# batra-mlp-lab/visdial

Measured on AMD Instinct MI355X. Metric: QA-rounds/sec training mn-att-ques-im-hist+disc (batch 20x10x100), higher is better.
Workload: dtype f32 operands and results; the option recurrence multiplies the EXACT 3-way bf16 split of both operands (9 bf16 MFMA products per fp32 product, f32 accumulate: fp32-grade, errors at the f32 MFMA's own level) -- its two step kernels and its weight-gradient contraction; f32 MFMA (v_mfma_f32_32x32x2_f32

## Files before the change

visdial_amd/csrc/gemm_ops.hip:

```cpp
#include "gemm_core.h"
#include "split_core.h"

using CfgBigDB = GemmCfg<4, 1, 4, 32>;
using CfgBig = GemmCfg<4, 1, 4, 16, 0, 3>;
using CfgSmall = GemmCfg<1, 4, 1, 32, 0, 3>;

static inline bool use_small(int M, int N) {
  return (long)vd_cdiv(M, CfgBig::BM) * vd_cdiv(N, CfgBig::BN) < 48;
}

static int check_align(const void* p, long ld, const char* what) {
  if (((uintptr_t)p & 15) != 0 || (ld & 3) != 0) {
    vd_set_error("%s: pointer must be 16-byte aligned and leading dimension a multiple of 4 (ld=%ld)", what, ld);
    return VD_ERR_ARG;
  }
  return VD_OK;
}

__global__ void colsum_kernel(const float* __restrict__ X, long ld, int M, int N, int rows_per_block,
                              float* __restrict__ out) {
  const int col = blockIdx.x * blockDim.x + threadIdx.x;
  if (col >= N) return;
  const int r0 = blockIdx.y * rows_per_block;
  const int r1 = min(M, r0 + rows_per_block);
// ... 69 lines not shown
  constexpr int TILE = 8192;
  char* const lds = reinterpret_cast<char*>(smem);
  const int wg = xcd_remap(blockIdx.x, gridDim.x);
  const int tile_n = wg % tiles_n, tile_m = (wg / tiles_n) % tiles_m, split = wg / (tiles_n * tiles_m);
  const int ks = split * kchunk, ke = min(K, ks + kchunk);
  const int nk = ke > ks ? (ke - ks) / 32 : 0;
  const int lane = threadIdx.x & 63;
  const int wm = __builtin_amdgcn_readfirstlane((int)threadIdx.x >> 6);
  const int m0 = tile_m * 128, n0 = tile_n * 128;

  f32x16 acc[4];
#pragma unroll
  for (int j = 0; j < 4; ++j)
#pragma unroll
    for (int r = 0; r < 16; ++r) acc[j][r] = 0.f;

  const int key = (lane & 7) >> 1, col = (lane >> 3) * 16 + (lane & 1) * 8;
  unsigned voffa[2], voffb[2];
#pragma unroll
  for (int i = 0; i < 2; ++i) {
    const int krow = (i * 4 + wm) * 4 + key;
    voffa[i] = (unsigned)(((long)krow * M + m0 + col) * 2);
    voffb[i] = (unsigned)(((long)krow * N + n0 + col) * 2);
  }
  const unsigned lds0 = (unsigned)(uintptr_t)lds;
  auto issue = [&](int kt, int buf) {
    const float* ak = reinterpret_cast<const float*>(A + (long)(ks + kt * 32) * M);
    const float* bk = reinterpret_cast<const float*>(B + (long)(ks + kt * 32) * N);
#pragma unroll
    for (int i = 0; i < 2; ++i) glds16(voffb[i], bk, lds0 + buf * 2 * TILE + TILE + (i * 4 + wm) * 1024);
#pragma unroll
    for (int i = 0; i < 2; ++i) glds16(voffa[i], ak, lds0 + buf * 2 * TILE + (i * 4 + wm) * 1024);
  };
  const int g = lane >> 4, li = lane & 15;
  const int frag = ((g >> 1) * 2) * 1024 + (g & 1) * 128 + li * 8;

  if (nk > 0) {
    issue(0, 0);
    if (nk > 1) issue(1, 1);
    int buf = 0;
    for (int kt = 0; kt < nk; ++kt) {
      if (kt + 1 < nk) asm volatile("s_waitcnt vmcnt(4)" ::: "memory");
      else asm volatile("s_waitcnt vmcnt(0)" ::: "memory");
      asm volatile("s_barrier" ::: "memory");
      if (kt + 2 < nk) issue(kt + 2, buf == 0 ? 2 : buf - 1);
      const char* ta = lds + buf * 2 * TILE;
      const char* tb = ta + TILE;
#pragma unroll
      for (int st = 0; st < 2; ++st) {
        const vd_bf16x8 a8 = tr_read8(ta, frag + st * 4096 + wm * 256);
        vd_bf16x8 b8[4];
#pragma unroll
        for (int j = 0; j < 4; ++j) b8[j] = tr_read8(tb, frag + st * 4096 + j * 256);
#pragma unroll
        for (int j = 0; j < 4; ++j) acc[j] = __builtin_amdgcn_mfma_f32_32x32x16_bf16(a8, b8[j], acc[j], 0, 0, 0);
      }
      buf = buf == 2 ? 0 : buf + 1;
    }
  }
#pragma unroll
  for (int j = 0; j < 4; ++j) {
    const int c = n0 + j * 32 + (lane & 31);
#pragma unroll
    for (int r = 0; r < 16; ++r) {
      const int row = m0 + wm * 32 + mfma_row(r, lane);
      unsafeAtomicAdd(C + (long)row * ldc + c, acc[j][r]);
    }
  }
}

template <int NBUF>
__global__ void __launch_bounds__(512)
gemm_bf16_tn_tr256_kernel(const vd_bf16_bits* __restrict__ A, const vd_bf16_bits* __restrict__ B, float* __restrict__ C, long ldc,
                          int M, int N, int K, int kchunk, int tiles_m, int tiles_n) {
  extern __shared__ __attribute__((aligned(16))) float smem[];
  constexpr int TILE = 16384;
  char* const lds = reinterpret_cast<char*>(smem);
  const int wg = xcd_remap(blockIdx.x, gridDim.x);
  const int tile_n = wg % tiles_n, tile_m = (wg / tiles_n) % tiles_m, split = wg / (tiles_n * tiles_m);
  const int ks = split * kchunk, ke = min(K, ks + kchunk);
  const int nk = ke > ks ? (ke - ks) / 32 : 0;
  const int lane = threadIdx.x & 63;
  const int w = __builtin_amdgcn_readfirstlane((int)threadIdx.x >> 6);
  const int wm = w & 3, wn = w >> 2;
  const int m0 = tile_m * 256, n0 = tile_n * 256;

  f32x16 acc[2][4];
#pragma unroll
  for (int i = 0; i < 2; ++i)
#pragma unroll
    for (int j = 0; j < 4; ++j)
#pragma unroll
      for (int r = 0; r < 16; ++r) acc[i][j][r] = 0.f;

  unsigned voffa[2], voffb[2];
#pragma unroll
  for (int i = 0; i < 2; ++i) {
    const int krow = (i * 8 + w) * 2 + (lane >> 5);
    const int cb = ((lane & 31) * 16) ^ ((krow & 3) << 6);
    voffa[i] = (unsigned)(((long)krow * M + m0) * 2 + cb);
    voffb[i] = (unsigned)(((long)krow * N + n0) * 2 + cb);
  }
  const unsigned lds0 = (unsigned)(uintptr_t)lds;
  auto issue = [&](int kt, int buf) {
    const float* ak = reinterpret_cast<const float*>(A + (long)(ks + kt * 32) * M);
    const float* bk = reinterpret_cast<const float*>(B + (long)(ks + kt * 32) * N);
#pragma unroll
    for (int i = 0; i < 2; ++i) glds16(voffb[i], bk, lds0 + buf * 2 * TILE + TILE + (i * 8 + w) * 1024);
#pragma unroll
    for (int i = 0; i < 2; ++i) glds16(voffa[i], ak, lds0 + buf * 2 * TILE + (i * 8 + w) * 1024);
  };
  const int g = lane >> 4, li = lane & 15;
  const int frag = (g >> 1) * 4096 + (li >> 2) * 512 + (g & 1) * 32 + (li & 3) * 8;
  int xa[2], xb[4];
#pragma unroll
  for (int i = 0; i < 2; ++i) xa[i] = frag + (((wm * 2 + i) ^ (li >> 2)) << 6);
#pragma unroll
  for (int j = 0; j < 4; ++j) xb[j] = frag + (((wn * 4 + j) ^ (li >> 2)) << 6);
  auto rd8 = [&](const char* base, int off) {
    typedef __attribute__((address_space(3))) vd_s16x4* lds_p;
    union {
      vd_s16x4 h[2];
      vd_bf16x8 v;
    } u;
    u.h[0] = __builtin_amdgcn_ds_read_tr16_b64_v4i16((lds_p)(base + off));
    u.h[1] = __builtin_amdgcn_ds_read_tr16_b64_v4i16((lds_p)(base + off + 2048));
    return u.v;
  };

  struct Frags {
    vd_bf16x8 a[2], b[4];
  };
  auto read_step = [&](Frags& f, int buf, int st) {
    const char* ta = lds + buf * 2 * TILE;
    const char* tb = ta + TILE;
#pragma unroll
    for (int i = 0; i < 2; ++i) f.a[i] = rd8(ta, xa[i] + st * 8192);
#pragma unroll
    for (int j = 0; j < 4; ++j) f.b[j] = rd8(tb, xb[j] + st * 8192);
  };
  auto mfma_step = [&](const Frags& f) {
#pragma unroll
    for (int i = 0; i < 2; ++i)
#pragma unroll
      for (int j = 0; j < 4; ++j) acc[i][j] = __builtin_amdgcn_mfma_f32_32x32x16_bf16(f.a[i], f.b[j], acc[i][j], 0, 0, 0);
  };
  auto wait_tiles_in_flight = [&](int later) {
    if (later >= 3) asm volatile("s_waitcnt vmcnt(12)" ::: "memory");
    else if (later == 2) asm volatile("s_waitcnt vmcnt(8)" ::: "memory");
    else if (later == 1) asm volatile("s_waitcnt vmcnt(4)" ::: "memory");
    else asm volatile("s_waitcnt vmcnt(0)" ::: "memory");
  };
  if (nk > 0) {
#pragma unroll
    for (int i = 0; i < NBUF - 1; ++i)
      if (i < nk) issue(i, i);
    wait_tiles_in_flight(min(NBUF - 2, nk - 1));
    asm volatile("s_barrier" ::: "memory");
    Frags f0, f1;
    read_step(f0, 0, 0);
    int buf = 0;
    for (int kt = 0; kt < nk; ++kt) {
      const int nbuf = buf == NBUF - 1 ? 0 : buf + 1;
      read_step(f1, buf, 1);
      mfma_step(f0);
      if (kt + 1 < nk) {
        wait_tiles_in_flight(min(NBUF - 3, nk - 2 - kt));
        asm volatile("s_barrier" ::: "memory");
        if (kt + NBUF - 1 < nk) issue(kt + NBUF - 1, buf == 0 ? NBUF - 1 : buf - 1);
        read_step(f0, nbuf, 0);
      }
      mfma_step(f1);
      buf = nbuf;
    }
  }
#pragma unroll
  for (int i = 0; i < 2; ++i)
#pragma unroll
    for (int j = 0; j < 4; ++j) {
      const int c = n0 + wn * 128 + j * 32 + (lane & 31);
#pragma unroll
      for (int r = 0; r < 16; ++r) {
        const int row = m0 + wm * 64 + i * 32 + mfma_row(r, lane);
        unsafeAtomicAdd(C + (long)row * ldc + c, acc[i][j][r]);
      }
    }
}

static int launch_gemm_bf16_tn_tr256(const vd_bf16_bits* A, const vd_bf16_bits* B, float* C, long ldc, int M, int N, int K,
                                     hipStream_t stream) {
  const int tiles_m = M / 256, tiles_n = N / 256;
  long splits = vd_cdiv(256, (long)tiles_m * tiles_n);
  int kchunk = vd_cdiv(vd_cdiv(K, splits), 32) * 32;
  if (kchunk < 32) kchunk = 32;
  splits = vd_cdiv(K, kchunk);
  static bool attr_set = false;
#ifndef VD_TR256_NBUF
#define VD_TR256_NBUF 3
#endif
  constexpr int NBUF = VD_TR256_NBUF;
  const int lds = NBUF * 2 * 16384;
  if (!attr_set) {
    VD_HIP(hipFuncSetAttribute(reinterpret_cast<const void*>(gemm_bf16_tn_tr256_kernel<NBUF>),
                               hipFuncAttributeMaxDynamicSharedMemorySize, lds));
    attr_set = true;
  }
  hipLaunchKernelGGL(gemm_bf16_tn_tr256_kernel<NBUF>, dim3((unsigned)(tiles_m * tiles_n * splits)), dim3(512), lds, stream, A, B, C,
                     ldc, M, N, K, kchunk, tiles_m, tiles_n);
  VD_LAUNCH_CHECK();
  return VD_OK;
}

static int launch_gemm_bf16_tn_tr(const vd_bf16_bits* A, const vd_bf16_bits* B, float* C, long ldc, int M, int N, int K,
                                  hipStream_t stream) {
  const int tiles_m = M / 128, tiles_n = N / 128;
  long splits = vd_cdiv(768, (long)tiles_m * tiles_n);
  int kchunk = vd_cdiv(vd_cdiv(K, splits), 32) * 32;
  if (kchunk < 32) kchunk = 32;
  splits = vd_cdiv(K, kchunk);
  static bool attr_set = false;
  const int lds = 3 * 2 * 8192;
  if (!attr_set) {
    VD_HIP(hipFuncSetAttribute(reinterpret_cast<const void*>(gemm_bf16_tn_tr_kernel),
                               hipFuncAttributeMaxDynamicSharedMemorySize, lds));
    attr_set = true;
  }
  hipLaunchKernelGGL(gemm_bf16_tn_tr_kernel, dim3((unsigned)(tiles_m * tiles_n * splits)), dim3(256), lds, stream, A, B, C,
                     ldc, M, N, K, kchunk, tiles_m, tiles_n);
  VD_LAUNCH_CHECK();
  return VD_OK;
}

extern "C" {

int vd_gemm_nt(const float* A, int64_t lda, const float* W, int64_t ldw, const float* bias, float* C,
               int64_t ldc, int M, int N, int K, int act, int accumulate, void* stream) {
  VD_CHECK_ARG(A && W && C && M >= 0 && N >= 0 && K >= 0 && K % 4 == 0, "vd_gemm_nt: bad args M=%d N=%d K=%d", M,
               N, K);
  if (int rc = check_align(A, lda, "vd_gemm_nt A")) return rc;
  if (int rc = check_align(W, ldw, "vd_gemm_nt W")) return rc;
  SrcRow a{A, lda}, b{W, ldw};
  hipStream_t s = (hipStream_t)stream;
  if (use_small(M, N)) {
    EpiStore<1> e{C, ldc, bias, act, accumulate};
    return launch_gemm<CfgSmall>(M, N, K, 1, a, b, e, s);
  }
  EpiStore<4> e{C, ldc, bias, act, accumulate};
  if (M >= 1024 && K >= 64 && K % 16 == 0 && (long)M * lda * 4 < (1L << 32) && (long)N * ldw * 4 < (1L << 32)) {
    int splits = 1;
    const long tiles = (long)vd_cdiv(M, 128) * vd_cdiv(N, 128);
    if (accumulate == 2 && !bias && act == VD_ACT_NONE && tiles < 512 && K >= 1024) {
      splits = (int)vd_cdiv(768, tiles);
      if (splits > K / 512) splits = K / 512;
    }
    return launch_gemm_glds<GemmCfg<4, 1, 4, 16, 0, 4, 41984>, false>(M, N, K, splits, A, lda, W, ldw, e, s, -1, splits > 1);
  }
  return launch_gemm<CfgBig>(M, N, K, 1, a, b, e, s);
}

int vd_gemm_nn(const float* A, int64_t lda, const float* B, int64_t ldb, const float* bias, float* C,
               int64_t ldc, int M, int N, int K, int accumulate, void* stream) {
  VD_CHECK_ARG(A && B && C && M >= 0 && N >= 0 && K >= 0 && (K % 4 == 0 || lda >= (K + 3) / 4 * 4) && N % 4 == 0,
               "vd_gemm_nn: bad args M=%d N=%d K=%d", M, N, K);
  if (int rc = check_align(A, lda, "vd_gemm_nn A")) return rc;
  if (int rc = check_align(B, ldb, "vd_gemm_nn B")) return rc;
  SrcRow a{A, lda};
  SrcK b{B, ldb};
  hipStream_t s = (hipStream_t)stream;
  if (use_small(M, N)) {
    EpiStore<1> e{C, ldc, bias, VD_ACT_NONE, accumulate};
    return launch_gemm<CfgSmall>(M, N, K, 1, a, b, e, s);
  }
  EpiStore<4> e{C, ldc, bias, VD_ACT_NONE, accumulate};
  return launch_gemm<CfgBig>(M, N, K, 1, a, b, e, s);
}

}

template <int NT>
struct EpiStoreLive : EpiStore<NT> {
  const int* tok_mask;
  static constexpr bool HAS_DEAD = true;
  __device__ __forceinline__ bool dead(int row_base, int ) const { return tok_mask[row_base] == 0; }
};
static_assert(CfgSmall::BM == VD_LSTM_FWD_TILE_SMALL && CfgBig::BM == VD_LSTM_FWD_TILE_BIG, "the projection's row tiles are the step kernels'");

int vd_gemm_nn_live_p(const float* A, int64_t lda, const float* B, int64_t ldb, const float* bias, float* C, int64_t ldc, int M, int N, int K,
                      const int32_t* tok_mask, int row_tile, hipStream_t s) {
  VD_CHECK_ARG(A && B && C && tok_mask && M >= 0 && N >= 0 && K >= 0 && (K % 4 == 0 || lda >= (K + 3) / 4 * 4) && N % 4 == 0 &&
                   (row_tile == CfgSmall::BM || row_tile == CfgBig::BM),
               "vd_gemm_nn (live rows): bad args M=%d N=%d K=%d row tile %d", M, N, K, row_tile);
  if (int rc = check_align(A, lda, "vd_gemm_nn (live rows) A")) return rc;
  if (int rc = check_align(B, ldb, "vd_gemm_nn (live rows) B")) return rc;
  SrcRow a{A, lda};
  SrcK b{B, ldb};
  if (row_tile == CfgSmall::BM) {
    EpiStoreLive<1> e{{C, ldc, bias, VD_ACT_NONE, 0}, tok_mask};
    return launch_gemm<CfgSmall>(M, N, K, 1, a, b, e, s);
  }
  EpiStoreLive<4> e{{C, ldc, bias, VD_ACT_NONE, 0}, tok_mask};
  return launch_gemm<CfgBig>(M, N, K, 1, a, b, e, s);
}

extern "C" {

int vd_gemm_tn_acc(const float* A, int64_t lda, const float* B, int64_t ldb, float* C, int64_t ldc, int M,
                   int N, int K, int flags, void* stream) {
  VD_CHECK_ARG(A && B && C && M >= 0 && N >= 0 && K >= 0 && (M % 4 == 0 || lda >= (M + 3) / 4 * 4) &&
                   (N % 4 == 0 || ldb >= (N + 3) / 4 * 4),
               "vd_gemm_tn_acc: bad args M=%d N=%d K=%d", M, N, K);
  if (int rc = check_align(A, lda, "vd_gemm_tn_acc A")) return rc;
  if (int rc = check_align(B, ldb, "vd_gemm_tn_acc B")) return rc;
  if (K == 0) return VD_OK;
  SrcK a{A, lda}, b{B, ldb};
  EpiAtomic<4> e{C, ldc};
  const long tiles = (long)vd_cdiv(M, CfgBig::BM) * vd_cdiv(N, CfgBig::BN);
  if ((flags & VD_FLAG_SPLIT9) && !(flags & VD_FLAG_BF16) && vd_tn_split_tiles(M, N) && K >= 8192 &&
      16L * lda * 4 < (1L << 31) && 16L * ldb * 4 < (1L << 31)) {
    const int K1 = K & ~15;
    if (int rc = launch_gemm_split_tn<9>(M, N, K1, A, lda, B, ldb, C, ldc, (hipStream_t)stream)) return rc;
    if (K1 == K) return VD_OK;
    SrcK a2{A + (long)K1 * lda, lda}, b2{B + (long)K1 * ldb, ldb};
    return launch_gemm<GemmCfg<4, 1, 4, 16, 0, 4, 41984>>(M, N, K - K1, 1, a2, b2, e, (hipStream_t)stream);
  }
  const bool kmaj = !(flags & VD_FLAG_BF16) && vd_tn_kmajor_fits(M, N, K);
  if (kmaj && K % 16 != 0) {
    const int K1 = K & ~15;
    if (int rc = vd_gemm_tn_acc(A, lda, B, ldb, C, ldc, M, N, K1, flags, stream)) return rc;
    SrcK a2{A + (long)K1 * lda, lda}, b2{B + (long)K1 * ldb, ldb};
    return launch_gemm<GemmCfg<4, 1, 4, 16, 0, 4, 41984>>(M, N, K - K1, 1, a2, b2, e, (hipStream_t)stream);
  }
  long splits = vd_cdiv(768, tiles);
  const long max_splits = vd_cdiv(K, 1024);
  if (splits > max_splits) splits = max_splits;
  if (splits < 1) splits = 1;
  if (flags & VD_FLAG_BF16) {
    if (M % 128 == 0 && N % 128 == 0 && K >= 32 && lda == M && ldb == N && (long)32 * N * 2 + 256 < (1L << 31)) {
      const vd_bf16_bits* a16 = vd_bf16_shadow_find(A, (size_t)K * M, VD_SHADOW_AT_BASE);
      const vd_bf16_bits* b16 = vd_bf16_shadow_find(B, (size_t)K * N, VD_SHADOW_AT_END);
      if (a16 && b16) {
        const int K1 = K & ~31;
        if (int rc = launch_gemm_bf16_tn_tr(a16, b16, C, ldc, M, N, K1, (hipStream_t)stream)) return rc;
        if (K1 == K) return VD_OK;
        SrcK a2{A + (long)K1 * lda, lda}, b2{B + (long)K1 * ldb, ldb};
        return launch_gemm<GemmCfg<4, 1, 4, 32, 0, 3, 0, 1>>(M, N, K - K1, 1, a2, b2, e, (hipStream_t)stream);
      }
    }
    if (vd_tn_split_tiles(M, N) && K >= 1024 && lda % 4 == 0 && ldb % 4 == 0 && 16L * lda * 4 < (1L << 31) &&
        16L * ldb * 4 < (1L << 31)) {
      const int K1 = K & ~15;
      if (int rc = launch_gemm_split_tn<1>(M, N, K1, A, lda, B, ldb, C, ldc, (hipStream_t)stream)) return rc;
      if (K1 == K) return VD_OK;
      SrcK a2{A + (long)K1 * lda, lda}, b2{B + (long)K1 * ldb, ldb};
      return launch_gemm<GemmCfg<4, 1, 4, 32, 0, 3, 0, 1>>(M, N, K - K1, 1, a2, b2, e, (hipStream_t)stream);
    }
    return launch_gemm<GemmCfg<4, 1, 4, 32, 0, 3, 0, 1>>(M, N, K, (int)splits, a, b, e, (hipStream_t)stream);
  }
  if (kmaj)
    return launch_gemm_glds<GemmCfg<4, 1, 4, 16, 0, 4, 41984>, true>(M, N, K, (int)splits, A, lda, B, ldb, e, (hipStream_t)stream, 0);
  return launch_gemm<GemmCfg<4, 1, 4, 16, 0, 4, 41984>>(M, N, K, (int)splits, a, b, e, (hipStream_t)stream);
}

int vd_gemm_tn_rows_acc(const float* A, int64_t lda, const int32_t* a_rows, const float* B, int64_t ldb,
                        const int32_t* b_rows, float* C, int64_t ldc, int M, int N, int K, void* stream) {
  VD_CHECK_ARG(A && B && C && a_rows && b_rows && M >= 0 && N >= 0 && K >= 0 && (M % 4 == 0 || lda >= (M + 3) / 4 * 4) &&
                   (N % 4 == 0 || ldb >= (N + 3) / 4 * 4),
               "vd_gemm_tn_rows_acc: bad args M=%d N=%d K=%d", M, N, K);
  if (int rc = check_align(A, lda, "vd_gemm_tn_rows_acc A")) return rc;
  if (int rc = check_align(B, ldb, "vd_gemm_tn_rows_acc B")) return rc;
  if (K == 0) return VD_OK;
  SrcKRows a{A, lda, a_rows}, b{B, ldb, b_rows};
  EpiAtomic<4> e{C, ldc};
  using Cfg = GemmCfg<4, 1, 4, 16, 0, 4, 41984>;
  const long tiles = (long)vd_cdiv(M, Cfg::BM) * vd_cdiv(N, Cfg::BN);
  long splits = vd_cdiv(768, tiles);
  const long max_splits = vd_cdiv(K, 1024);
  if (splits > max_splits) splits = max_splits;
  if (splits < 1) splits = 1;
  return launch_gemm<Cfg>(M, N, K, (int)splits, a, b, e, (hipStream_t)stream);
}

int vd_colsum_acc(const float* X, int64_t ld, int M, int N, float* out, void* stream) {
  VD_CHECK_ARG(X && out && M >= 0 && N >= 0, "vd_colsum_acc: bad args");
  if (M == 0 || N == 0) return VD_OK;
  if (N % 4 == 0 && ld % 4 == 0 && ((uintptr_t)X & 15) == 0 && M >= 64) {
    const int cb4 = vd_cdiv(N, 256);
    int rb4 = vd_cdiv(2048, cb4);
    int rpb = vd_cdiv(vd_cdiv(M, rb4), 4) * 4;
    if (rpb < 32) rpb = 32;
    rb4 = vd_cdiv(M, rpb);
    hipLaunchKernelGGL(colsum4_kernel, dim3(cb4, rb4), dim3(256), 0, (hipStream_t)stream, X, ld, M, N, rpb, out);
    VD_LAUNCH_CHECK();
    return VD_OK;
  }
  const int cb = vd_cdiv(N, 256);
  int rb = vd_cdiv(1024, cb);
  int rows_per_block = vd_cdiv(M, rb);
  if (rows_per_block < 16) rows_per_block = 16;
  rb = vd_cdiv(M, rows_per_block);
  hipLaunchKernelGGL(colsum_kernel, dim3(cb, rb), dim3(256), 0, (hipStream_t)stream, X, ld, M, N,
                     rows_per_block, out);
  VD_LAUNCH_CHECK();
  return VD_OK;
}

}

int vd_gemm_tn_live_grouped(const VdLiveProduct* prod, int nprod, const int32_t* items, const int32_t* chunk_start, int chunks,
                            hipStream_t stream) {
  using Cfg = GemmCfg<4, 1, 4, 16, 0, 4, 41984>;
  VD_CHECK_ARG(prod && nprod >= 1 && nprod <= VD_LIVE_MAXP && items && chunk_start && chunks >= 0, "vd_gemm_tn_live_grouped: bad args");
  LiveGroupArgs<VD_LIVE_MAXP> g{};
  for (int i = 0; i < nprod; ++i) {
    const VdLiveProduct& p = prod[i];
    VD_CHECK_ARG(p.A && p.B && p.C && p.segs && p.M > 0 && p.N > 0 && p.M % Cfg::BM == 0 && p.N % Cfg::BN == 0 && p.lda >= p.M && p.ldb >= p.N &&
                     16 * p.lda * 4 < (1L << 31) && 16 * p.ldb * 4 < (1L << 31) && p.ldc < (1L << 31) &&
                     (long)(p.M / Cfg::BM) * (p.N / Cfg::BN) < (1 << 24),
                 "vd_gemm_tn_live_grouped: product %d: M=%d N=%d", i, p.M, p.N);
    if (int rc = check_align(p.A, p.lda, "vd_gemm_tn_live_grouped A")) return rc;
    if (int rc = check_align(p.B, p.ldb, "vd_gemm_tn_live_grouped B")) return rc;
    g.p[i] = LiveProduct{p.A, p.B, p.C, reinterpret_cast<const int4*>(p.segs), (int)p.lda, (int)p.ldb, (int)p.ldc, p.N / Cfg::BN};
  }
  g.items = reinterpret_cast<const int4*>(items);
  g.chunk_start = chunk_start;
  return launch_live_grouped<Cfg, VD_LIVE_MAXP>(g, chunks, stream);
}

__global__ void __launch_bounds__(256) bf16_tn_tail_kernel(const vd_bf16_bits* __restrict__ A, const vd_bf16_bits* __restrict__ B, float* __restrict__ C,
                                                           long ldc, int M, int N, int K) {
  const long i = (long)blockIdx.x * 256 + threadIdx.x;
  if (i >= (long)M * N) return;
  const int m = (int)(i / N), n = (int)(i % N);
  float acc = 0.f;
  for (int k = 0; k < K; ++k)
    acc += __uint_as_float((unsigned)A[(long)k * M + m] << 16) * __uint_as_float((unsigned)B[(long)k * N + n] << 16);
  unsafeAtomicAdd(C + (long)m * ldc + n, acc);
}
int vd_gemm_tn_acc_bf16(const vd_bf16_bits* A16, const vd_bf16_bits* B16, float* C, int64_t ldc, int M, int N, int K, hipStream_t stream) {
  VD_CHECK_ARG(A16 && B16 && C && M % 128 == 0 && N % 128 == 0 && K >= 0, "vd_gemm_tn_acc_bf16: M, N must be multiples of 128");
  const int K1 = K & ~31;
  if (K1 > 0) {
    const bool big = M % 256 == 0 && N % 256 == 0 && K1 >= 8192;
    if (int rc = big ? launch_gemm_bf16_tn_tr256(A16, B16, C, ldc, M, N, K1, stream) : launch_gemm_bf16_tn_tr(A16, B16, C, ldc, M, N, K1, stream)) return rc;
  }
  if (K1 < K) {
    hipLaunchKernelGGL(bf16_tn_tail_kernel, dim3((unsigned)(((long)M * N + 255) / 256)), dim3(256), 0, stream, A16 + (long)K1 * M, B16 + (long)K1 * N,
                       C, (long)ldc, M, N, K - K1);
    VD_LAUNCH_CHECK();
  }
  return VD_OK;
}
```

visdial_amd/csrc/split_core.h:

```cpp
#pragma once
#include "gemm_core.h"
#include "paths.h"

typedef __bf16 vd_bf16x8 __attribute__((ext_vector_type(8)));

__device__ __forceinline__ unsigned vd_cvt_pk_bf16(float a, float b) {
  unsigned r;
  asm("v_cvt_pk_bf16_f32 %0, %1, %2" : "=v"(r) : "v"(a), "v"(b));
  return r;
}
__device__ __forceinline__ float vd_bf16_lo_f32(unsigned p) {
  float r;
  asm("v_lshlrev_b32 %0, 16, %1" : "=v"(r) : "v"(p));
  return r;
}
__device__ __forceinline__ float vd_bf16_hi_f32(unsigned p) {
  float r;
  asm("v_and_b32 %0, 0xffff0000, %1" : "=v"(r) : "v"(p));
  return r;
}
__device__ __forceinline__ float vd_sub_f32(float a, float b) {
  float r;
  asm("v_sub_f32 %0, %1, %2" : "=v"(r) : "v"(a), "v"(b));
  return r;
}
__device__ __forceinline__ void vd_split3_pair(float a, float b, unsigned& hi, unsigned& mid, unsigned& lo) {
  hi = vd_cvt_pk_bf16(a, b);
  const float ra = vd_sub_f32(a, vd_bf16_lo_f32(hi)), rb = vd_sub_f32(b, vd_bf16_hi_f32(hi));
  mid = vd_cvt_pk_bf16(ra, rb);
  lo = vd_cvt_pk_bf16(vd_sub_f32(ra, vd_bf16_lo_f32(mid)), vd_sub_f32(rb, vd_bf16_hi_f32(mid)));
}

typedef unsigned vd_u32x4 __attribute__((ext_vector_type(4)));
__device__ __forceinline__ void vd_split3(const float4& u, const float4& w, vd_bf16x8& hi, vd_bf16x8& mid, vd_bf16x8& lo) {
  unsigned h[4], m[4], l[4];
  vd_split3_pair(u.x, u.y, h[0], m[0], l[0]);
  vd_split3_pair(u.z, u.w, h[1], m[1], l[1]);
  vd_split3_pair(w.x, w.y, h[2], m[2], l[2]);
  vd_split3_pair(w.z, w.w, h[3], m[3], l[3]);
  hi = __builtin_bit_cast(vd_bf16x8, (vd_u32x4){h[0], h[1], h[2], h[3]});
  mid = __builtin_bit_cast(vd_bf16x8, (vd_u32x4){m[0], m[1], m[2], m[3]});
  lo = __builtin_bit_cast(vd_bf16x8, (vd_u32x4){l[0], l[1], l[2], l[3]});
}

static __global__ void __launch_bounds__(256) f32_to_bf16x3_kernel(const float* __restrict__ src, vd_bf16_bits* __restrict__ dst, long n4, long plane) {
  const long i = (long)blockIdx.x * 256 + threadIdx.x;
  if (i >= n4) return;
  const float4 v = reinterpret_cast<const float4*>(src)[i];
  float4 r1, r2;
  typedef __bf16 bf4 __attribute__((ext_vector_type(4)));
  const bf4 h = {(__bf16)v.x, (__bf16)v.y, (__bf16)v.z, (__bf16)v.w};
  r1.x = v.x - (float)h[0]; r1.y = v.y - (float)h[1]; r1.z = v.z - (float)h[2]; r1.w = v.w - (float)h[3];
  const bf4 m = {(__bf16)r1.x, (__bf16)r1.y, (__bf16)r1.z, (__bf16)r1.w};
  r2.x = r1.x - (float)m[0]; r2.y = r1.y - (float)m[1]; r2.z = r1.z - (float)m[2]; r2.w = r1.w - (float)m[3];
  const bf4 l = {(__bf16)r2.x, (__bf16)r2.y, (__bf16)r2.z, (__bf16)r2.w};
  *reinterpret_cast<bf4*>(dst + i * 4) = h;
  *reinterpret_cast<bf4*>(dst + plane + i * 4) = m;
  *reinterpret_cast<bf4*>(dst + 2 * plane + i * 4) = l;
}
static int weights_to_bf16x3(const float* src, vd_bf16_bits* dst, long n, hipStream_t s) {
  hipLaunchKernelGGL(f32_to_bf16x3_kernel, dim3((unsigned)((n / 4 + 255) / 256)), dim3(256), 0, s, src, dst, n / 4, n);
  VD_LAUNCH_CHECK();
  return VD_OK;
}

struct SplitCfg {
    static constexpr int NT = 4, WM = 4, THREADS = 64 * WM;
  static constexpr int BM = 32 * WM, BN = 128, KS = 32;
  static constexpr int BTILE = BN * 64;
  static constexpr int STAGE = 3 * BTILE;
  static constexpr int LDS_BYTES = 2 * STAGE;
  static constexpr int SCR = LDS_BYTES / WM / 4;
  static_assert(SCR >= 32 * QUAD_LD, "quad_to_tile's 32 rows of QUAD_LD floats");
};

#ifndef VD_SPLIT_CG
#define VD_SPLIT_CG 2
#endif
static_assert(VD_SPLIT_CG >= 1 && VD_SPLIT_CG <= 8 && 8 % VD_SPLIT_CG == 0, "the XCD grid is VD_SPLIT_CG x (8 / VD_SPLIT_CG)");
__device__ __forceinline__ bool split_tile_of(int bid, int nwg, int tiles_m, int tiles_n, int& tile_m, int& tile_n) {
  constexpr int CG = VD_SPLIT_CG, RG = 8 / CG;
  if ((tiles_n % CG) == 0 && tiles_n >= 8) {
    const int xcd = bid & 7, li = bid >> 3, cpg = tiles_n / CG, rpg = (tiles_m + RG - 1) / RG;
    tile_n = (xcd % CG) * cpg + li % cpg;
    tile_m = (xcd / CG) * rpg + li / cpg;
    return tile_m < tiles_m && li / cpg < rpg;
  }
  const int wg = xcd_remap(bid, nwg);
  tile_n = wg % tiles_n;
  tile_m = wg / tiles_n;
  return true;
}
__device__ __forceinline__ int split_swz(int q) { return (0x78 >> (2 * (q & 3))) & 3; }
static int split_grid(int tiles_m, int tiles_n) {
  constexpr int CG = VD_SPLIT_CG, RG = 8 / CG;
  if ((tiles_n % CG) == 0 && tiles_n >= 8) return 8 * ((tiles_m + RG - 1) / RG) * (tiles_n / CG);
  return tiles_m * tiles_n;
}

template <int NPROD, class Epi>
__global__ void __launch_bounds__(SplitCfg::THREADS, 3)
gemm_split_kernel(int M, int N, int K, int tiles_n, const float* A, long lda, const vd_bf16_bits* B, long ldb, long bplane, Epi epi) {
  using Cfg = SplitCfg;
  constexpr int NT = Cfg::NT;
  extern __shared__ __attribute__((aligned(16))) float smem[];
  int tile_m, tile_n;
  if (!split_tile_of((int)blockIdx.x, (int)gridDim.x, (M + Cfg::BM - 1) / Cfg::BM, tiles_n, tile_m, tile_n)) return;
  const int row_base = tile_m * Cfg::BM, col_base = tile_n * Cfg::BN;
  constexpr int NIB = 24 / Cfg::WM;
  const int tid = (int)threadIdx.x, lane = tid & 63;
  const int wm = __builtin_amdgcn_readfirstlane(tid >> 6);
  const int nfull = K / 32, nm = nfull + ((K >> 4) & 1);
  const int wrow = row_base + wm * 32;
  const int g = lane >> 4, l15 = lane & 15;

  vd_f32x4 acc[2][2 * NT];
#pragma unroll
  for (int rt = 0; rt < 2; ++rt)
#pragma unroll
    for (int j = 0; j < 2 * NT; ++j)
#pragma unroll
      for (int r = 0; r < 4; ++r) acc[rt][j][r] = 0.f;

  typename EpiPreOf<Epi>::type pre;
  if constexpr (EpiPreOf<Epi>::value) epi.preload(pre, wrow, lane, M);

  unsigned aoff[2];
#pragma unroll
  for (int rt = 0; rt < 2; ++rt) aoff[rt] = (unsigned)(((long)min(wrow + rt * 16 + l15, M - 1) * lda + g * 8) * 4);
  float4 an[2][2];
  auto load_a = [&](int m) {
    const char* ak = reinterpret_cast<const char*>(A + (long)m * 32);
    const bool live = m < nfull || g < 2;
#pragma unroll
    for (int rt = 0; rt < 2; ++rt) {
      an[rt][0] = an[rt][1] = make_float4(0.f, 0.f, 0.f, 0.f);
      if (live) {
        an[rt][0] = *reinterpret_cast<const float4*>(ak + aoff[rt]);
        an[rt][1] = *reinterpret_cast<const float4*>(ak + aoff[rt] + 16);
      }
    }
  };
  const int csrc = (lane & 3) ^ split_swz(lane >> 4);
  unsigned voffb[NIB];
#pragma unroll
  for (int i = 0; i < NIB; ++i) {
    const int r = ((wm * NIB + i) & 7) * 16 + (lane >> 2);
    voffb[i] = (unsigned)(((long)min(col_base + r, N - 1) * ldb + csrc * 8) * 2);
  }
  const unsigned lds0 = (unsigned)(uintptr_t)smem;
  auto issue_b = [&](int m, int st) {
    const unsigned back = m < nfull ? 0u : (unsigned)(csrc >> 1) * 32u;
#pragma unroll
    for (int i = 0; i < NIB; ++i) {
      const int q = wm * NIB + i;
      glds16(voffb[i] - back, reinterpret_cast<const float*>(B + (long)(q >> 3) * bplane + (long)m * 32), lds0 + st * Cfg::STAGE + q * 1024);
    }
  };
  const int bfrag = l15 * 64 + ((g ^ split_swz(l15 >> 2)) * 16);

  auto load_a_full = [&](int m) {
    const char* ak = reinterpret_cast<const char*>(A + (long)m * 32);
#pragma unroll
    for (int rt = 0; rt < 2; ++rt) {
      an[rt][0] = *reinterpret_cast<const float4*>(ak + aoff[rt]);
      an[rt][1] = *reinterpret_cast<const float4*>(ak + aoff[rt] + 16);
    }
  };
  auto issue_b_full = [&](int m, int st) {
#pragma unroll
    for (int i = 0; i < NIB; ++i) {
      const int q = wm * NIB + i;
      glds16(voffb[i], reinterpret_cast<const float*>(B + (long)(q >> 3) * bplane + (long)m * 32), lds0 + st * Cfg::STAGE + q * 1024);
    }
  };

  auto step = [&](int m, int st, auto full_next) {
    vd_bf16x8 ap[2][3];
#pragma unroll
    for (int rt = 0; rt < 2; ++rt) vd_split3(an[rt][0], an[rt][1], ap[rt][0], ap[rt][1], ap[rt][2]);
    __builtin_amdgcn_sched_barrier(0);
    asm volatile("s_waitcnt vmcnt(0)" ::: "memory");
    asm volatile("s_barrier" ::: "memory");
    if constexpr (decltype(full_next)::value) {
      issue_b_full(m + 1, st ^ 1);
      load_a_full(m + 1);
    } else if (m + 1 < nm) {
      issue_b(m + 1, st ^ 1);
      load_a(m + 1);
    }
    __builtin_amdgcn_sched_barrier(0);
    const char* sbase = reinterpret_cast<const char*>(smem) + st * Cfg::STAGE + bfrag;
#pragma unroll
    for (int p = 2; p >= 0; --p)
#pragma unroll
      for (int jh = 0; jh < 2; ++jh) {
        vd_bf16x8 bp[NT];
#pragma unroll
        for (int j = 0; j < NT; ++j) {
          const vd_f32x4 t = *reinterpret_cast<const vd_f32x4*>(sbase + p * Cfg::BTILE + (jh * NT + j) * 1024);
          bp[j] = __builtin_bit_cast(vd_bf16x8, t);
        }
#pragma unroll
        for (int i = 2; i >= 0; --i) {
          constexpr int LIM = NPROD >= 9 ? 4 : NPROD >= 6 ? 2 : NPROD >= 3 ? 1 : 0;
          if (i + p > LIM) continue;
#pragma unroll
          for (int rt = 0; rt < 2; ++rt)
#pragma unroll
            for (int j = 0; j < NT; ++j)
              acc[rt][jh * NT + j] = __builtin_amdgcn_mfma_f32_16x16x32_bf16(ap[rt][i], bp[j], acc[rt][jh * NT + j], 0, 0, 0);
        }
      }
    asm volatile("s_waitcnt lgkmcnt(0)\n\ts_barrier" ::: "memory");
  };
  if (nm > 0) {
    issue_b(0, 0);
    load_a(0);
    int m = 0;
    for (; m + 1 < nfull; ++m) step(m, m & 1, std::true_type{});
    if (m < nm) {
      step(m, m & 1, std::false_type{});
      if (++m < nm) step(m, m & 1, std::false_type{});
    }
  }
  float* scr = smem + wm * Cfg::SCR;
  f32x16 tile[NT];
#pragma unroll
  for (int j = 0; j < NT; ++j) tile[j] = quad_to_tile(acc[0][2 * j], acc[0][2 * j + 1], acc[1][2 * j], acc[1][2 * j + 1], scr, lane);
  if constexpr (EpiPreOf<Epi>::value) epi(tile, wrow, col_base, lane, M, N, scr, &pre);
  else epi(tile, wrow, col_base, lane, M, N, scr);
}

template <int NPROD, class Epi>
static int launch_gemm_split(int M, int N, int K, const float* A, long lda, const vd_bf16_bits* B, long ldb, long bplane, const Epi& e,
                             hipStream_t stream) {
  if (M <= 0 || N <= 0) return VD_OK;
  using Cfg = SplitCfg;
  VD_CHECK_ARG(K % 16 == 0 && lda % 4 == 0 && ldb % 8 == 0 && (long)M * lda * 4 < (1L << 32) && (long)N * ldb * 2 < (1L << 32),
               "launch_gemm_split: unsupported shape M=%d N=%d K=%d", M, N, K);
  const int tiles_m = vd_cdiv(M, Cfg::BM), tiles_n = vd_cdiv(N, Cfg::BN);
  auto kern = gemm_split_kernel<NPROD, Epi>;
  static bool attr_set = false;
  if (!attr_set) {
    VD_HIP(hipFuncSetAttribute(reinterpret_cast<const void*>(kern), hipFuncAttributeMaxDynamicSharedMemorySize, 160 * 1024));
    attr_set = true;
  }
  hipLaunchKernelGGL(kern, dim3(split_grid(tiles_m, tiles_n)), dim3(Cfg::THREADS), Cfg::LDS_BYTES, stream, M, N, K, tiles_n, A, lda, B, ldb, bplane, e);
  VD_LAUNCH_CHECK();
  return VD_OK;
}

template <class Epi>
static int launch_gemm_split(int nprod, int M, int N, int K, const float* A, long lda, const vd_bf16_bits* B, long ldb, long bplane,
                             const Epi& e, hipStream_t stream) {
  if (nprod == 9) return launch_gemm_split<9>(M, N, K, A, lda, B, ldb, bplane, e, stream);
  if (nprod == 6) return launch_gemm_split<6>(M, N, K, A, lda, B, ldb, bplane, e, stream);
  return launch_gemm_split<3>(M, N, K, A, lda, B, ldb, bplane, e, stream);
}

struct SplitTnCfg {
  static constexpr int BM = 256, BN = 128, THREADS = 256;
  static constexpr int ATILE = 16 * BM * 4;
  static constexpr int BTILE = 16 * BN * 4;
  static constexpr int STAGE = ATILE + BTILE;
  static constexpr int LDS_BYTES = 2 * STAGE;
};
static_assert(SplitTnCfg::BM == VD_SPLIT_TN_BM && SplitTnCfg::BN == VD_SPLIT_TN_BN, "paths.h vd_tn_split_tiles");

template <int NPROD>
__global__ void __launch_bounds__(256, 2)
gemm_split_tn_kernel(int M, int N, int kchunk, int K, int tiles, int tiles_n, int splits, const float* A, long lda, const float* B, long ldb,
                     float* C, long ldc) {
  using Cfg = SplitTnCfg;
  extern __shared__ __attribute__((aligned(16))) float smem[];
  int tile, split;
  if ((splits & 7) == 0) {
    const int xcd = (int)blockIdx.x & 7, li = (int)blockIdx.x >> 3;
    split = xcd * (splits >> 3) + li / tiles;
    tile = li % tiles;
  } else {
    split = (int)blockIdx.x / tiles;
    tile = (int)blockIdx.x % tiles;
  }
  const int m_base = (tile / tiles_n) * Cfg::BM, n_base = (tile % tiles_n) * Cfg::BN;
  const int ks = split * kchunk, ke = min(K, ks + kchunk);
  const int nm = ke > ks ? (ke - ks) / 16 : 0;
  const int tid = (int)threadIdx.x, lane = tid & 63;
  const int wm = __builtin_amdgcn_readfirstlane(tid >> 6);

  f32x16 acc[2][4];
#pragma unroll
  for (int mb = 0; mb < 2; ++mb)
#pragma unroll
    for (int j = 0; j < 4; ++j)
#pragma unroll
      for (int r = 0; r < 16; ++r) acc[mb][j][r] = 0.f;

  unsigned voffa[4], voffb[2];
#pragma unroll
  for (int i = 0; i < 4; ++i) voffa[i] = (unsigned)(((long)(wm * 4 + i) * lda + m_base + lane * 4) * 4);
#pragma unroll
  for (int i = 0; i < 2; ++i) voffb[i] = (unsigned)(((long)((wm * 2 + i) * 2 + (lane >> 5)) * ldb + n_base + (lane & 31) * 4) * 4);
  const unsigned lds0 = (unsigned)(uintptr_t)smem;
  auto issue = [&](int m, int st) {
    const unsigned base = lds0 + st * Cfg::STAGE;
    const float* ak = A + (long)(ks + m * 16) * lda;
    const float* bk = B + (long)(ks + m * 16) * ldb;
#pragma unroll
    for (int i = 0; i < 2; ++i) glds16(voffb[i], bk, base + Cfg::ATILE + (wm * 2 + i) * 1024);
#pragma unroll
    for (int i = 0; i < 4; ++i) glds16(voffa[i], ak, base + (wm * 4 + i) * 1024);
  };
  const int hi = lane >> 5, l31 = lane & 31;

  int mb1 = 32;
  asm("" : "+v"(mb1));
  const float* sA0 = smem + (hi * 8) * Cfg::BM + wm * 64 + l31;
  const float* sA1 = sA0 + mb1;
  const float* sB0 = smem + Cfg::ATILE / 4 + (hi * 8) * Cfg::BN + l31;
  auto step = [&](int m, auto stage) {
    constexpr int st = decltype(stage)::value;
    if (m + 1 < nm) {
      issue(m + 1, st ^ 1);
      asm volatile("s_waitcnt vmcnt(6)" ::: "memory");
    } else {
      asm volatile("s_waitcnt vmcnt(0)" ::: "memory");
    }
    asm volatile("s_barrier" ::: "memory");
    const float* sB = sB0 + st * (Cfg::STAGE / 4);
    vd_bf16x8 ap[2][3], bp[2][3];
    auto load_b = [&](int j, vd_bf16x8 (&dst)[3]) {
      const float* p = sB + j * 32;
      const float4 u = make_float4(p[0], p[Cfg::BN], p[2 * Cfg::BN], p[3 * Cfg::BN]);
      const float4 w = make_float4(p[4 * Cfg::BN], p[5 * Cfg::BN], p[6 * Cfg::BN], p[7 * Cfg::BN]);
      vd_split3(u, w, dst[0], dst[1], dst[2]);
    };
#pragma unroll
    for (int mb = 0; mb < 2; ++mb) {
      const float* p = (mb ? sA1 : sA0) + st * (Cfg::STAGE / 4);
      const float4 u = make_float4(p[0], p[Cfg::BM], p[2 * Cfg::BM], p[3 * Cfg::BM]);
      const float4 w = make_float4(p[4 * Cfg::BM], p[5 * Cfg::BM], p[6 * Cfg::BM], p[7 * Cfg::BM]);
      vd_split3(u, w, ap[mb][0], ap[mb][1], ap[mb][2]);
    }
    load_b(0, bp[0]);
#pragma unroll
    for (int j = 0; j < 4; ++j) {
      __builtin_amdgcn_sched_barrier(0);
      if (j + 1 < 4) load_b(j + 1, bp[(j + 1) & 1]);
#pragma unroll
      for (int pb = 2; pb >= 0; --pb)
#pragma unroll
        for (int pa = 2; pa >= 0; --pa) {
          constexpr int LIM = NPROD >= 9 ? 4 : NPROD >= 6 ? 2 : NPROD >= 3 ? 1 : 0;
          if (pa + pb > LIM) continue;
#pragma unroll
          for (int mb = 0; mb < 2; ++mb) acc[mb][j] = __builtin_amdgcn_mfma_f32_32x32x16_bf16(ap[mb][pa], bp[j & 1][pb], acc[mb][j], 0, 0, 0);
        }
      if (j + 1 < 4) {
        __builtin_amdgcn_sched_group_barrier(0x100, 4, 0);
#pragma unroll
        for (int i = 0; i < 18; ++i) {
          __builtin_amdgcn_sched_group_barrier(0x008, 1, 0);
          __builtin_amdgcn_sched_group_barrier(0x002, 4, 0);
        }
      }
    }
    asm volatile("s_waitcnt lgkmcnt(0)\n\ts_barrier" ::: "memory");
  };
  if (nm > 0) {
    issue(0, 0);
    int m = 0;
    for (; m + 1 < nm; m += 2) {
      step(m, std::integral_constant<int, 0>{});
      step(m + 1, std::integral_constant<int, 1>{});
    }
    if (m < nm) step(m, std::integral_constant<int, 0>{});
  }
  if (nm == 0) return;
  const EpiAtomic<4> e{C, ldc};
#pragma unroll
  for (int mb = 0; mb < 2; ++mb) e(acc[mb], m_base + wm * 64 + mb * 32, n_base, lane, M, N);
}

template <int NPROD>
static int launch_gemm_split_tn(int M, int N, int K, const float* A, long lda, const float* B, long ldb, float* C, long ldc, hipStream_t stream) {
  using Cfg = SplitTnCfg;
  VD_CHECK_ARG(M % Cfg::BM == 0 && N % Cfg::BN == 0 && K % 16 == 0 && lda % 4 == 0 && ldb % 4 == 0 && 16L * lda * 4 < (1L << 31) && 16L * ldb * 4 < (1L << 31),
               "launch_gemm_split_tn: unsupported shape M=%d N=%d K=%d", M, N, K);
  if (K == 0) return VD_OK;
  const int tiles_n = N / Cfg::BN, tiles = (M / Cfg::BM) * tiles_n;
  int splits = vd_cdiv(2L * vd_num_cus(), tiles);
  splits = (splits + 7) & ~7;
  int kchunk = vd_cdiv(vd_cdiv(K, splits), 16) * 16;
  if (kchunk < 64) kchunk = 64;
  splits = vd_cdiv(K, kchunk);
  if (splits >= 8) splits = (splits + 7) & ~7;
  auto kern = gemm_split_tn_kernel<NPROD>;
  static bool attr_set = false;
  if (!attr_set) {
    VD_HIP(hipFuncSetAttribute(reinterpret_cast<const void*>(kern), hipFuncAttributeMaxDynamicSharedMemorySize, 160 * 1024));
    attr_set = true;
  }
  hipLaunchKernelGGL(kern, dim3(tiles * splits), dim3(256), Cfg::LDS_BYTES, stream, M, N, kchunk, K, tiles, tiles_n, splits, A, lda, B, ldb, C, ldc);
  VD_LAUNCH_CHECK();
  return VD_OK;
}
```

Measured before the change: 9514.

## Pre-split B tile into bf16 planes once per stage in split TN kernel

The split-TN weight-gradient kernel used to have every warp re-split the fp32 B fragments into three bf16 planes on each read. Now each warp splits only its own quarter of the next stage's B tile once and writes the bf16 planes to LDS, so the MFMA loop just loads ready planes. The A split for the second row block is interleaved between MFMAs, and the pipeline prologue and epilogue are restructured around this. It also adds a per-device LDS-attribute cache and an exported entry point. The cost is extra LDS writes and more LDS use per stage (56 KB for nine products), plus more complex wait and barrier ordering.

```diff
diff --git a/visdial_amd/csrc/gemm_ops.hip b/visdial_amd/csrc/gemm_ops.hip
--- a/visdial_amd/csrc/gemm_ops.hip
+++ b/visdial_amd/csrc/gemm_ops.hip
@@ -395,6 +395,16 @@
   return launch_gemm<CfgBig>(M, N, K, 1, a, b, e, s);
 }
 
+int vd_gemm_split_tn_p(const float* A, int64_t lda, const float* B, int64_t ldb, float* C, int64_t ldc, int M, int N, int K, int nprod,
+                       hipStream_t stream) {
+  VD_CHECK_ARG(A && B && C && M > 0 && N > 0 && K >= 0 && (nprod == 9 || nprod == 1), "vd_gemm_split_tn_p: bad args M=%d N=%d K=%d nprod=%d",
+               M, N, K, nprod);
+  if (int rc = check_align(A, lda, "vd_gemm_split_tn_p A")) return rc;
+  if (int rc = check_align(B, ldb, "vd_gemm_split_tn_p B")) return rc;
+  if (nprod == 9) return launch_gemm_split_tn<9>(M, N, K, A, lda, B, ldb, C, ldc, stream);
+  return launch_gemm_split_tn<1>(M, N, K, A, lda, B, ldb, C, ldc, stream);
+}
+
 extern "C" {
 
 int vd_gemm_tn_acc(const float* A, int64_t lda, const float* B, int64_t ldb, float* C, int64_t ldc, int M,
diff --git a/visdial_amd/csrc/split_core.h b/visdial_amd/csrc/split_core.h
--- a/visdial_amd/csrc/split_core.h
+++ b/visdial_amd/csrc/split_core.h
@@ -61,6 +61,16 @@
 static int weights_to_bf16x3(const float* src, vd_bf16_bits* dst, long n, hipStream_t s) {
   hipLaunchKernelGGL(f32_to_bf16x3_kernel, dim3((unsigned)((n / 4 + 255) / 256)), dim3(256), 0, s, src, dst, n / 4, n);
   VD_LAUNCH_CHECK();
+  return VD_OK;
+}
+
+constexpr int SPLIT_ATTR_DEVS = 64;
+static int split_lds_attr(const void* kern, bool (&done)[SPLIT_ATTR_DEVS]) {
+  int dev = 0;
+  VD_HIP(hipGetDevice(&dev));
+  if (dev >= 0 && dev < SPLIT_ATTR_DEVS && done[dev]) return VD_OK;
+  VD_HIP(hipFuncSetAttribute(kern, hipFuncAttributeMaxDynamicSharedMemorySize, 160 * 1024));
+  if (dev >= 0 && dev < SPLIT_ATTR_DEVS) done[dev] = true;
   return VD_OK;
 }
 
@@ -241,11 +251,8 @@
                "launch_gemm_split: unsupported shape M=%d N=%d K=%d", M, N, K);
   const int tiles_m = vd_cdiv(M, Cfg::BM), tiles_n = vd_cdiv(N, Cfg::BN);
   auto kern = gemm_split_kernel<NPROD, Epi>;
-  static bool attr_set = false;
-  if (!attr_set) {
-    VD_HIP(hipFuncSetAttribute(reinterpret_cast<const void*>(kern), hipFuncAttributeMaxDynamicSharedMemorySize, 160 * 1024));
-    attr_set = true;
-  }
+  static bool attr_set[SPLIT_ATTR_DEVS] = {};
+  if (const int rc = split_lds_attr(reinterpret_cast<const void*>(kern), attr_set)) return rc;
   hipLaunchKernelGGL(kern, dim3(split_grid(tiles_m, tiles_n)), dim3(Cfg::THREADS), Cfg::LDS_BYTES, stream, M, N, K, tiles_n, A, lda, B, ldb, bplane, e);
   VD_LAUNCH_CHECK();
   return VD_OK;
@@ -262,17 +269,24 @@
 struct SplitTnCfg {
   static constexpr int BM = 256, BN = 128, THREADS = 256;
   static constexpr int ATILE = 16 * BM * 4;
-  static constexpr int BTILE = 16 * BN * 4;
-  static constexpr int STAGE = ATILE + BTILE;
-  static constexpr int LDS_BYTES = 2 * STAGE;
+  static constexpr int BQUART = 16 * 32 * 4;
+  static constexpr int nplanes(int nprod) { return nprod >= 6 ? 3 : nprod >= 3 ? 2 : 1; }
+  static constexpr int bblock(int nprod) { return nplanes(nprod) * 1024 > BQUART ? nplanes(nprod) * 1024 : BQUART; }
+  static constexpr int stage(int nprod) { return ATILE + 4 * bblock(nprod); }
+  static constexpr int lds_bytes(int nprod) { return 2 * stage(nprod); }
+  static constexpr int LDS_BYTES = 2 * (ATILE + 4 * 3 * 1024);
+  static constexpr int SIDE_LDS = 41 * 1024;
 };
 static_assert(SplitTnCfg::BM == VD_SPLIT_TN_BM && SplitTnCfg::BN == VD_SPLIT_TN_BN, "paths.h vd_tn_split_tiles");
+static_assert(SplitTnCfg::LDS_BYTES == SplitTnCfg::lds_bytes(9) && SplitTnCfg::lds_bytes(1) == 48 * 1024, "nine products: 56 KB; one: 48 KB");
+static_assert(2 * SplitTnCfg::LDS_BYTES + SplitTnCfg::SIDE_LDS <= 160 * 1024, "the side lane's workgroups must fit beside two of these");
 
 template <int NPROD>
 __global__ void __launch_bounds__(256, 2)
 gemm_split_tn_kernel(int M, int N, int kchunk, int K, int tiles, int tiles_n, int splits, const float* A, long lda, const float* B, long ldb,
                      float* C, long ldc) {
   using Cfg = SplitTnCfg;
+  constexpr int NPL = Cfg::nplanes(NPROD), BBLK = Cfg::bblock(NPROD), STAGE = Cfg::stage(NPROD);
   extern __shared__ __attribute__((aligned(16))) float smem[];
   int tile, split;
   if ((splits & 7) == 0) {
@@ -301,14 +315,14 @@
 #pragma unroll
   for (int i = 0; i < 4; ++i) voffa[i] = (unsigned)(((long)(wm * 4 + i) * lda + m_base + lane * 4) * 4);
 #pragma unroll
-  for (int i = 0; i < 2; ++i) voffb[i] = (unsigned)(((long)((wm * 2 + i) * 2 + (lane >> 5)) * ldb + n_base + (lane & 31) * 4) * 4);
+  for (int i = 0; i < 2; ++i) voffb[i] = (unsigned)(((long)(i * 8 + (lane >> 3)) * ldb + n_base + wm * 32 + (lane & 7) * 4) * 4);
   const unsigned lds0 = (unsigned)(uintptr_t)smem;
   auto issue = [&](int m, int st) {
-    const unsigned base = lds0 + st * Cfg::STAGE;
+    const unsigned base = lds0 + st * STAGE;
     const float* ak = A + (long)(ks + m * 16) * lda;
     const float* bk = B + (long)(ks + m * 16) * ldb;
 #pragma unroll
-    for (int i = 0; i < 2; ++i) glds16(voffb[i], bk, base + Cfg::ATILE + (wm * 2 + i) * 1024);
+    for (int i = 0; i < 2; ++i) glds16(voffb[i], bk, base + Cfg::ATILE + wm * BBLK + i * 1024);
 #pragma unroll
     for (int i = 0; i < 4; ++i) glds16(voffa[i], ak, base + (wm * 4 + i) * 1024);
   };
@@ -318,70 +332,131 @@
   asm("" : "+v"(mb1));
   const float* sA0 = smem + (hi * 8) * Cfg::BM + wm * 64 + l31;
   const float* sA1 = sA0 + mb1;
-  const float* sB0 = smem + Cfg::ATILE / 4 + (hi * 8) * Cfg::BN + l31;
-  auto step = [&](int m, auto stage) {
-    constexpr int st = decltype(stage)::value;
-    if (m + 1 < nm) {
-      issue(m + 1, st ^ 1);
-      asm volatile("s_waitcnt vmcnt(6)" ::: "memory");
-    } else {
-      asm volatile("s_waitcnt vmcnt(0)" ::: "memory");
-    }
-    asm volatile("s_barrier" ::: "memory");
-    const float* sB = sB0 + st * (Cfg::STAGE / 4);
+  const float* sBq = smem + (Cfg::ATILE + wm * BBLK) / 4 + (hi * 8) * 32 + l31;
+  const char* sBp = reinterpret_cast<const char*>(smem) + Cfg::ATILE + lane * 16;
+  constexpr int LIM = NPROD >= 9 ? 4 : NPROD >= 6 ? 2 : NPROD >= 3 ? 1 : 0;
+  auto read_own = [&](int st, float4& u, float4& w) {
+    const float* p = sBq + st * (STAGE / 4);
+    u = make_float4(p[0], p[32], p[2 * 32], p[3 * 32]);
+    w = make_float4(p[4 * 32], p[5 * 32], p[6 * 32], p[7 * 32]);
+  };
+  auto write_own = [&](int st, const float4& u, const float4& w) {
+    vd_bf16x8 own[3];
+    vd_split3(u, w, own[0], own[1], own[2]);
+    char* d = const_cast<char*>(sBp) + st * STAGE + wm * BBLK;
+#pragma unroll
+    for (int pl = 0; pl < NPL; ++pl) *reinterpret_cast<vd_bf16x8*>(d + pl * 1024) = own[pl];
+  };
+  auto step = [&](int m, auto stage, auto has_next) {
+    const int st = stage, other = st ^ 1;
+    constexpr bool next = decltype(has_next)::value;
+    if constexpr (next) issue(m + 1, st ^ 1);
     vd_bf16x8 ap[2][3], bp[2][3];
+    float4 au[2], aw[2], u, w;
+#pragma unroll
+    for (int mb = 0; mb < 2; ++mb) {
+      const float* q = (mb ? sA1 : sA0) + st * (STAGE / 4);
+      au[mb] = make_float4(q[0], q[Cfg::BM], q[2 * Cfg::BM], q[3 * Cfg::BM]);
+      aw[mb] = make_float4(q[4 * Cfg::BM], q[5 * Cfg::BM], q[6 * Cfg::BM], q[7 * Cfg::BM]);
+    }
+    const char* sP = sBp + st * STAGE;
     auto load_b = [&](int j, vd_bf16x8 (&dst)[3]) {
-      const float* p = sB + j * 32;
-      const float4 u = make_float4(p[0], p[Cfg::BN], p[2 * Cfg::BN], p[3 * Cfg::BN]);
-      const float4 w = make_float4(p[4 * Cfg::BN], p[5 * Cfg::BN], p[6 * Cfg::BN], p[7 * Cfg::BN]);
-      vd_split3(u, w, dst[0], dst[1], dst[2]);
+#pragma unroll
+      for (int pl = 0; pl < NPL; ++pl) dst[pl] = *reinterpret_cast<const vd_bf16x8*>(sP + j * BBLK + pl * 1024);
     };
-#pragma unroll
-    for (int mb = 0; mb < 2; ++mb) {
-      const float* p = (mb ? sA1 : sA0) + st * (Cfg::STAGE / 4);
-      const float4 u = make_float4(p[0], p[Cfg::BM], p[2 * Cfg::BM], p[3 * Cfg::BM]);
-      const float4 w = make_float4(p[4 * Cfg::BM], p[5 * Cfg::BM], p[6 * Cfg::BM], p[7 * Cfg::BM]);
-      vd_split3(u, w, ap[mb][0], ap[mb][1], ap[mb][2]);
-    }
     load_b(0, bp[0]);
-#pragma unroll
-    for (int j = 0; j < 4; ++j) {
+    __builtin_amdgcn_sched_barrier(0);
+    vd_split3(au[0], aw[0], ap[0][0], ap[0][1], ap[0][2]);
+    __builtin_amdgcn_sched_barrier(0);
+    {
+      unsigned h[4], md[4], lo[4];
+      auto pair = [&](int i) {
+        vd_split3_pair(i == 0 ? au[1].x : i == 1 ? au[1].z : i == 2 ? aw[1].x : aw[1].z, i == 0 ? au[1].y : i == 1 ? au[1].w : i == 2 ? aw[1].y : aw[1].w,
+                       h[i], md[i], lo[i]);
+      };
+      int idx = 0;
+#pragma unroll
+      for (int pb = 2; pb >= 0; --pb)
+#pragma unroll
+        for (int pa = 2; pa >= 0; --pa) {
+          if (pa + pb > LIM) continue;
+          acc[0][0] = __builtin_amdgcn_mfma_f32_32x32x16_bf16(ap[0][pa], bp[0][pb], acc[0][0], 0, 0, 0);
+          if (idx < 4) {
+            __builtin_amdgcn_sched_barrier(0);
+            pair(idx);
+            if (idx == 3) load_b(1, bp[1]);
+            __builtin_amdgcn_sched_barrier(0);
+          }
+          ++idx;
+        }
+#pragma unroll
+      for (int i = idx; i < 4; ++i) pair(i);
+      if (idx < 4) load_b(1, bp[1]);
+      ap[1][0] = __builtin_bit_cast(vd_bf16x8, (vd_u32x4){h[0], h[1], h[2], h[3]});
+      ap[1][1] = __builtin_bit_cast(vd_bf16x8, (vd_u32x4){md[0], md[1], md[2], md[3]});
+      ap[1][2] = __builtin_bit_cast(vd_bf16x8, (vd_u32x4){lo[0], lo[1], lo[2], lo[3]});
       __builtin_amdgcn_sched_barrier(0);
-      if (j + 1 < 4) load_b(j + 1, bp[(j + 1) & 1]);
 #pragma unroll
       for (int pb = 2; pb >= 0; --pb)
 #pragma unroll
         for (int pa = 2; pa >= 0; --pa) {
-          constexpr int LIM = NPROD >= 9 ? 4 : NPROD >= 6 ? 2 : NPROD >= 3 ? 1 : 0;
+          if (pa + pb > LIM) continue;
+          acc[1][0] = __builtin_amdgcn_mfma_f32_32x32x16_bf16(ap[1][pa], bp[0][pb], acc[1][0], 0, 0, 0);
+        }
+    }
+#pragma unroll
+    for (int j = 1; j < 4; ++j) {
+      __builtin_amdgcn_sched_barrier(0);
+      if (j + 1 < 4) {
+        load_b(j + 1, bp[(j + 1) & 1]);
+      } else if constexpr (next) {
+        asm volatile("s_waitcnt vmcnt(4)" ::: "memory");
+        read_own(other, u, w);
+      }
+#pragma unroll
+      for (int pb = 2; pb >= 0; --pb)
+#pragma unroll
+        for (int pa = 2; pa >= 0; --pa) {
           if (pa + pb > LIM) continue;
 #pragma unroll
           for (int mb = 0; mb < 2; ++mb) acc[mb][j] = __builtin_amdgcn_mfma_f32_32x32x16_bf16(ap[mb][pa], bp[j & 1][pb], acc[mb][j], 0, 0, 0);
         }
       if (j + 1 < 4) {
+        __builtin_amdgcn_sched_group_barrier(0x100, NPL, 0);
+      } else if constexpr (next) {
+        write_own(other, u, w);
         __builtin_amdgcn_sched_group_barrier(0x100, 4, 0);
-#pragma unroll
-        for (int i = 0; i < 18; ++i) {
-          __builtin_amdgcn_sched_group_barrier(0x008, 1, 0);
-          __builtin_amdgcn_sched_group_barrier(0x002, 4, 0);
-        }
+        __builtin_amdgcn_sched_group_barrier(0x008, LIM >= 4 ? 14 : 1, 0);
+        __builtin_amdgcn_sched_group_barrier(0x200, NPL, 0);
       }
     }
-    asm volatile("s_waitcnt lgkmcnt(0)\n\ts_barrier" ::: "memory");
+    asm volatile("s_waitcnt vmcnt(0) lgkmcnt(0)\n\ts_barrier" ::: "memory");
   };
   if (nm > 0) {
+    const std::integral_constant<int, 0> s0{};
+    const std::integral_constant<int, 1> s1{};
     issue(0, 0);
+    asm volatile("s_waitcnt vmcnt(4)" ::: "memory");
+    float4 u, w;
+    read_own(0, u, w);
+    write_own(0, u, w);
+    asm volatile("s_waitcnt vmcnt(0) lgkmcnt(0)\n\ts_barrier" ::: "memory");
     int m = 0;
-    for (; m + 1 < nm; m += 2) {
-      step(m, std::integral_constant<int, 0>{});
-      step(m + 1, std::integral_constant<int, 1>{});
-    }
-    if (m < nm) step(m, std::integral_constant<int, 0>{});
+    for (; m + 2 < nm; m += 2) {
+      step(m, s0, std::true_type{});
+      step(m + 1, s1, std::true_type{});
+    }
+    if (m + 2 == nm) step(m++, s0, std::true_type{});
+    step(m, m & 1, std::false_type{});
   }
   if (nm == 0) return;
   const EpiAtomic<4> e{C, ldc};
 #pragma unroll
   for (int mb = 0; mb < 2; ++mb) e(acc[mb], m_base + wm * 64 + mb * 32, n_base, lane, M, N);
 }
+
+int vd_gemm_split_tn_p(const float* A, int64_t lda, const float* B, int64_t ldb, float* C, int64_t ldc, int M, int N, int K, int nprod,
+                       hipStream_t stream);
 
 template <int NPROD>
 static int launch_gemm_split_tn(int M, int N, int K, const float* A, long lda, const float* B, long ldb, float* C, long ldc, hipStream_t stream) {
@@ -397,12 +472,9 @@
   splits = vd_cdiv(K, kchunk);
   if (splits >= 8) splits = (splits + 7) & ~7;
   auto kern = gemm_split_tn_kernel<NPROD>;
-  static bool attr_set = false;
-  if (!attr_set) {
-    VD_HIP(hipFuncSetAttribute(reinterpret_cast<const void*>(kern), hipFuncAttributeMaxDynamicSharedMemorySize, 160 * 1024));
-    attr_set = true;
-  }
-  hipLaunchKernelGGL(kern, dim3(tiles * splits), dim3(256), Cfg::LDS_BYTES, stream, M, N, kchunk, K, tiles, tiles_n, splits, A, lda, B, ldb, C, ldc);
+  static bool attr_set[SPLIT_ATTR_DEVS] = {};
+  if (const int rc = split_lds_attr(reinterpret_cast<const void*>(kern), attr_set)) return rc;
+  hipLaunchKernelGGL(kern, dim3(tiles * splits), dim3(256), Cfg::lds_bytes(NPROD), stream, M, N, kchunk, K, tiles, tiles_n, splits, A, lda, B, ldb, C, ldc);
   VD_LAUNCH_CHECK();
   return VD_OK;
 }
```

Measured after the change: 9749, median of 6. 2.5% higher.
